# junejunejune/c_orb_slam

Measured on AMD Instinct MI355X. Metric: tracking FPS + ORB matches/sec, KITTI-00 stereo; local-BA iter/sec, higher is better.
Workload: dtype u8

## Files before the change

### c_orb_slam_amd/csrc/ba.hpp

```cpp
#pragma once
#include <functional>
#include <hip/hip_runtime.h>

#include <cstdint>
#include <future>
#include <vector>

#include "../../include/orbslam_gpu.h"
#include "ba_struct.hpp"
#include "ba_struct_gpu.hpp"
#include "ba_types.hpp"
#include "comm.hpp"
#include "ldlt.hpp"
#include "orb_common.hpp"

namespace orbgpu {

constexpr int kBaTiledMinPoses = 24;

struct Se3 {
    double q[4];
    double t[3];
    double pad;
};
// ... 146 lines not shown
struct PoseProbDev;
class PoseEngine {
public:
    ~PoseEngine();
    int init();
    int run(int count, const pose_problem* P, float* Tcw_out, uint8_t* const* outlier, int* ninliers);
    int run_device(int count, const pose_problem* P, float* const* Tcw_out, uint8_t* const* outlier, int* ninliers);
    int run_frames_device(int count, const pose_frame* F, float* const* Tcw_out, uint8_t* const* outlier,
                          int* ninliers, hipStream_t s = nullptr, DeferredChain* chain = nullptr);
    hipStream_t stream() const { return stream_; }
    void set_timing(bool on) { timing_ = on; }
    int last_timing(float* ms);

private:
    int launch_device(int count, const int* Ns, const std::function<void(int, PoseProbDev&)>& fill,
                      float* const* Tcw_out, uint8_t* const* outlier, int* ninliers, hipStream_t s = nullptr,
                      DeferredChain* chain = nullptr);
    hipStream_t stream_ = nullptr;
    void* dArena_ = nullptr;
    void* hArena_ = nullptr;
    size_t cap_ = 0;
    hipEvent_t lastUse_ = nullptr;
    bool lastUseSet_ = false;
    bool timing_ = false, timed_ = false;
    hipEvent_t tA_ = nullptr, tB_ = nullptr;
};

int debug_ldlt(int n, const double* S, const double* b, double* x, int variant);
int debug_csum(const double* v, int n, double* out);
int debug_ldlt_factor(int n, const double* S, double* out);
int debug_wave_tree(const double* v64, double* out);
int debug_shared_div(const double* a, const double* b, int n, double* out);
int debug_set_csum_lds_max(int v);
int debug_set_scale_small_max(int v);
int debug_set_struct_gpu_min_edges(int v);
int debug_set_posegraph_check(int on);
int debug_prof(unsigned long long* out32);

}
```

### c_orb_slam_amd/csrc/capi_match.cpp

```cpp
#include <cstring>
#include <new>
#include <vector>

#include "capi_handles.hpp"

using orbgpu::FrameDev;
using orbgpu::Matcher;
using orbgpu::SearchDev;


namespace {

size_t al(size_t n) { return (n + 255) & ~(size_t)255; }

template <class T>
T* up(Matcher* m, const T* src, size_t count, hipStream_t s, int* err) {
    if (!src || count == 0) return nullptr;
    void* d = m->arena_alloc(count * sizeof(T));
    if (!d || hipMemcpyAsync(d, src, count * sizeof(T), hipMemcpyHostToDevice, s) != hipSuccess) {
        *err = ORB_E_HIP;
        return nullptr;
    }
    return (T*)d;
}
// ... 319 lines not shown
        f.projX = proj_x[p];
        f.projXR = proj_xr[p];
        f.projY = proj_y[p];
        f.level = level[p];
        f.viewCos = view_cos[p];
        f.mpIndex = (int*)m->arena_alloc((size_t)std::max(maps[p].n, 1) * 4);
        f.nvisible = d_nv + p;
        if (!f.mpIndex) return ORB_E_HIP;
    }
    if (err) return err;
    if (m->frustum(probs, fr, viewingCosLimit, logScaleFactor)) return ORB_E_HIP;
    if (hipMemcpyAsync(nvisible, d_nv, (size_t)count * 4, hipMemcpyDeviceToHost, s) != hipSuccess) return ORB_E_HIP;
    return orbgpu::stream_wait(s) == hipSuccess ? ORB_OK : ORB_E_HIP;
}

int ORBmatcher_SearchLocalPoints_batch(ORBmatcher_h h, int count, const orb_frame* F, int32_t* const* cur_mp,
                                       const orb_localmap* maps, float logScaleFactor, float th, float nnratio,
                                       int* nmatches, int* nvisible) {
    if (!h || count < 0 || (count > 0 && (!F || !cur_mp || !maps || !nmatches || !nvisible))) return ORB_E_INVALID;
    if (count == 0) return ORB_OK;
    Matcher* m = h->m;
    if (!m->device_pointers()) return ORB_E_INVALID;
    hipStream_t s = m->stream();
    size_t need = al((size_t)count * 8) + al(sizeof(orbgpu::FrustumDev) * count) + 4096;
    for (int p = 0; p < count; p++) {
        const orb_localmap& M = maps[p];
        if (!frame_ok(&F[p]) || !F[p].Tcw || M.n < 0 || !cur_mp[p]) return ORB_E_INVALID;
        if (M.n > 0 && (!M.pos || !M.desc || !M.observations || !M.max_dist || !M.min_dist || !M.normal || !M.skip))
            return ORB_E_INVALID;
        need += 7 * al((size_t)M.n * 4) + 256;
    }
    if (m->arena_reserve(need)) return ORB_E_HIP;
    int err = 0;
    int* d_cnt = (int*)m->count_buf((size_t)count * 8);
    if (!d_cnt) return ORB_E_HIP;
    if (hipMemsetAsync(d_cnt, 0, (size_t)count * 8, s) != hipSuccess) return ORB_E_HIP;
    std::vector<SearchDev> probs(count);
    std::vector<orbgpu::FrustumDev> fr(count);
    for (int p = 0; p < count; p++) {
        SearchDev& P = probs[p];
        memset(&P, 0, sizeof(P));
        P.cur = frame_dev(m, &F[p], true, s, &err);
        P.nq = maps[p].n;
        P.mpPos = maps[p].pos;
        P.mpDesc = maps[p].desc;
        P.mpObs = maps[p].observations;
        P.curMP = cur_mp[p];
        P.nmatches = d_cnt + p;
        orbgpu::FrustumDev& f = fr[p];
        memset(&f, 0, sizeof(f));
        f.maxDist = maps[p].max_dist;
        f.minDist = maps[p].min_dist;
        f.normal = maps[p].normal;
        f.skip = maps[p].skip;
        f.nvisible = d_cnt + count + p;
    }
    if (err) return err;
    const int rc = m->search_local_points(probs, fr, 0.5f, logScaleFactor, th, nnratio > 0.f ? nnratio : m->nnratio());
    if (rc) return rc == -1 ? ORB_E_INVALID : ORB_E_HIP;
    if (m->d2h_counts(nmatches, d_cnt, (size_t)count * 4) || m->d2h_counts(nvisible, d_cnt + count, (size_t)count * 4))
        return ORB_E_HIP;
    (void)s;
    return m->end_call() ? ORB_E_HIP : ORB_OK;
}

int ORBmatcher_SearchDense_batch(ORBmatcher_h h, int count, const uint8_t* const* qdesc, const int* nq,
                                 const uint8_t* const* tdesc, const int* nt, int32_t* const* best_idx,
                                 int32_t* const* best_dist, int32_t* const* second_dist) {
    if (!h || count < 0 || (count > 0 && (!qdesc || !nq || !tdesc || !nt || !best_idx || !best_dist || !second_dist)))
        return ORB_E_INVALID;
    for (int p = 0; p < count; p++) {
        if (nq[p] < 0 || nt[p] < 0) return ORB_E_INVALID;
        if (nq[p] > 0 && (!qdesc[p] || !best_idx[p] || !best_dist[p] || !second_dist[p])) return ORB_E_INVALID;
        if (nt[p] > 0 && !tdesc[p]) return ORB_E_INVALID;
    }
    if (count == 0) return ORB_OK;
    Matcher* m = h->m;
    const bool dev = m->device_pointers();
    hipStream_t s = m->stream();
    std::vector<orbgpu::DenseDev> probs;
    if (!dev) {
        size_t need = 4096;
// ... 89 lines not shown
```

### c_orb_slam_amd/csrc/capi_stereo.cpp

```cpp
#include <algorithm>
#include <cmath>
#include <cstring>
#include <vector>

#include "capi_handles.hpp"
#include "stereo.hpp"

namespace {
size_t al(size_t n) { return (n + 255) & ~(size_t)255; }

template <class T>
T* up(orbgpu::Matcher* m, const T* src, size_t count, hipStream_t s, int* err) {
    if (!src || count == 0) return nullptr;
    void* d = m->arena_alloc(count * sizeof(T));
    if (!d || hipMemcpyAsync(d, src, count * sizeof(T), hipMemcpyHostToDevice, s) != hipSuccess) {
        *err = ORB_E_HIP;
        return nullptr;
    }
    return (T*)d;
}
}

extern "C" {

// ... 15 lines not shown
        !keysR || !descR || !uRight || !depth || !nmatches)
        return ORB_E_INVALID;
    if (npairs == 0) return ORB_OK;
    const orbgpu::Extractor* EL = left->ex;
    const orbgpu::Extractor* ER = right->ex;
    if (!EL->pyramid_base() || !ER->pyramid_base() || first_left + npairs > EL->last_batch() ||
        first_right + npairs > ER->last_batch())
        return ORB_E_INVALID;
    const auto& LL = EL->levels();
    const auto& LR = ER->levels();
    if (LL.size() != LR.size() || (int)LL.size() > orbgpu::kStereoMaxLevels) return ORB_E_INVALID;
    for (size_t l = 0; l < LL.size(); l++)
        if (LL[l].w != LR[l].w || LL[l].h != LR[l].h || LL[l].pitch != LR[l].pitch || LL[l].off != LR[l].off)
            return ORB_E_INVALID;
    if (!(mb > 0.0f)) return ORB_E_INVALID;
    for (int p = 0; p < npairs; p++) {
        if (NL[p] < 0 || NR[p] < 0 || NL[p] > orbgpu::kStereoMaxKeys || NR[p] > 65535) return ORB_E_INVALID;
        if ((NL[p] && (!keysL[p] || !descL[p] || !uRight[p] || !depth[p])) || (NR[p] && (!keysR[p] || !descR[p])))
            return ORB_E_INVALID;
    }
    orbgpu::Matcher* m = h->m;
    const bool dev = m->device_pointers();
    hipStream_t s = m->stream();
    if (orbgpu::stream_wait(EL->stream()) != hipSuccess ||
        (ER != EL && orbgpu::stream_wait(ER->stream()) != hipSuccess))
        return ORB_E_HIP;
    orbgpu::StereoParams P;
    std::memset(&P, 0, sizeof(P));
    for (size_t l = 0; l < LL.size(); l++) {
        P.lv[l].off = (long long)LL[l].off;
        P.lv[l].pitch = LL[l].pitch;
        P.lv[l].w = LL[l].w;
        P.lv[l].h = LL[l].h;
        P.scale[l] = EL->scale()[l];
        P.invScale[l] = EL->inv_scale()[l];
    }
    P.mbf = mbf;
    P.mb = mb;
    P.rows0 = LL[0].h;
    if (P.rows0 > orbgpu::kStereoMaxRows) return ORB_E_INVALID;
    const int band = (int)std::ceil(4.0f * EL->scale()[LL.size() - 1]) + 3;
    size_t need = al(sizeof(orbgpu::StereoDev) * npairs) + al(4 * (size_t)npairs);
    int maxNL = 0;
    for (int p = 0; p < npairs; p++) {
        need += al(4 * (size_t)NL[p]) + al(4 * ((size_t)P.rows0 + 1)) + al(8 * (size_t)NR[p] * band + 8);
        if (!dev) need += al(28 * (size_t)NL[p]) + al(32 * (size_t)NL[p]) + al(28 * (size_t)NR[p]) +
                          al(32 * (size_t)NR[p]) + 2 * al(4 * (size_t)NL[p]);
        maxNL = std::max(maxNL, NL[p]);
// ... 240 lines not shown
```

### c_orb_slam_amd/csrc/orb_common.hpp

```cpp
#pragma once
#include <hip/hip_runtime.h>
#include <cstdint>
#include <cstdio>
#include <cstring>
#include <deque>
#include <mutex>
#include <vector>

#define ORB_HIP_CHECK(expr)                                                            \
    do {                                                                               \
        hipError_t _e = (expr);                                                        \
        if (_e != hipSuccess) {                                                        \
            fprintf(stderr, "[orbslam_gpu] HIP error %s at %s:%d: %s\n",               \
                    hipGetErrorName(_e), __FILE__, __LINE__, #expr);                   \
            return -2;                                                                 \
        }                                                                              \
    } while (0)

namespace orbgpu {

hipError_t stream_wait(hipStream_t s);

class DeferredChain {
public:
    ~DeferredChain() {
        for (auto& b : blocks_) (void)hipHostFree(b.p);
        for (auto& b : devs_) (void)hipFree(b.p);
        for (auto& e : events_)
            if (e.ev) (void)hipEventDestroy(e.ev);
    }
    bool on() const { return on_; }
    void set(bool v) { on_ = v; }
    void* stage(const void* src, size_t bytes) {
        void* p = take(bytes);
        if (p && bytes) std::memcpy(p, src, bytes);
        return p;
    }
    void* land(void* user, size_t bytes) {
        void* p = take(bytes);
        if (p) cur_outs_.push_back(Out{p, user, bytes});
        return p;
    }
    void* dev_counts(size_t bytes) {
        bytes = (bytes + 255) & ~(size_t)255;
        std::lock_guard<std::mutex> g(mu_);
        if (cur_dev_ < 0 || devs_[cur_dev_].used + bytes > devs_[cur_dev_].cap) {
            int k = -1;
            for (size_t q = 0; q < devs_.size(); q++)
                if (!devs_[q].busy && devs_[q].cap >= bytes) {
                    k = (int)q;
                    break;
                }
            if (k < 0) {
                void* p = nullptr;
                const size_t cap = bytes < 65536 ? 65536 : bytes;
                if (hipMalloc(&p, cap) != hipSuccess) return nullptr;
                devs_.push_back(DevBlock{p, cap, 0, false});
                k = (int)devs_.size() - 1;
            }
            devs_[k].busy = true;
            devs_[k].used = 0;
            cur_devs_.push_back(k);
            cur_dev_ = k;
        }
        DevBlock& b = devs_[cur_dev_];
        void* p = (char*)b.p + b.used;
        b.used += bytes;
        return p;
    }
    void land_dev(void* user, const void* dev, size_t bytes) {
        std::lock_guard<std::mutex> g(mu_);
        cur_dev_outs_.push_back(DevOut{user, dev, bytes});
    }
    int close(hipStream_t s, long long* id) {
        std::vector<int> devs;
        std::vector<DevOut> douts;
        std::vector<DevBlock> snap;
        {
            std::lock_guard<std::mutex> g(mu_);
            devs.swap(cur_devs_);
            douts.swap(cur_dev_outs_);
            cur_dev_ = -1;
            for (int k : devs) snap.push_back(devs_[k]);
        }
        bool ok = true;
        std::vector<Out> mapped;
        for (const DevBlock& b : snap) {
            if (!b.used) continue;
            char* pin = (char*)take(b.used);
            if (!pin || hipMemcpyAsync(pin, b.p, b.used, hipMemcpyDeviceToHost, s) != hipSuccess) {
                ok = false;
                break;
            }
            for (const DevOut& o : douts)
                if ((const char*)o.dev >= (const char*)b.p && (const char*)o.dev < (const char*)b.p + b.cap)
                    mapped.push_back(Out{pin + ((const char*)o.dev - (const char*)b.p), o.user, o.bytes});
        }
        std::lock_guard<std::mutex> g(mu_);
        size_t k = 0;
        if (ok) {
            while (k < events_.size() && (events_[k].live || events_[k].waiters > 0)) k++;
            if (k == events_.size()) {
                events_.push_back(Ev{});
                ok = hipEventCreateWithFlags(&events_[k].ev, hipEventDisableTiming) == hipSuccess;
            }
            ok = ok && hipEventRecord(events_[k].ev, s) == hipSuccess;
        }
        if (!ok) {
            fprintf(stderr, "[orbslam_gpu] deferred chain: closing the epoch failed; its counts are lost\n");
            (void)hipStreamSynchronize(s);
            for (int d : devs) devs_[d].busy = false;
            for (int b : cur_blocks_) blocks_[b].busy = false;
            cur_blocks_.clear();
            cur_outs_.clear();
            failed_ = true;
            return -2;
        }
        for (auto& o : mapped) cur_outs_.push_back(o);
        events_[k].live = true;
// ... 61 lines not shown

private:
    struct Block {
        void* p;
        size_t cap;
        bool busy;
    };
    struct Out {
        void* pin;
        void* user;
        size_t bytes;
    };
    struct Epoch {
        long long id;
        int ev;
        std::vector<int> blocks;
        std::vector<Out> outs;
        std::vector<int> devs;
    };
    struct DevBlock {
        void* p;
        size_t cap, used;
        bool busy;
    };
    struct DevOut {
        void* user;
        const void* dev;
        size_t bytes;
    };
    struct Ev {
        hipEvent_t ev = nullptr;
        bool live = false;
        int waiters = 0;
    };
    void* take(size_t bytes) {
        bytes = (bytes + 255) & ~(size_t)255;
        std::lock_guard<std::mutex> g(mu_);
        for (size_t k = 0; k < blocks_.size(); k++)
            if (!blocks_[k].busy && blocks_[k].cap >= bytes) {
                blocks_[k].busy = true;
                cur_blocks_.push_back((int)k);
                return blocks_[k].p;
            }
        void* p = nullptr;
        const size_t cap = bytes < 65536 ? 65536 : bytes;
        if (hipHostMalloc(&p, cap) != hipSuccess) return nullptr;
// ... 162 lines not shown
```

### c_orb_slam_amd/csrc/orb_extract.hip

```cpp
#include "orb_extract.hpp"

#include <algorithm>
#include <atomic>
#include <chrono>
#include <cmath>
#include <cstring>
#include <thread>

namespace orbgpu {

__constant__ int8_t c_pattern[256 * 4];
__constant__ int8_t c_disc[2 * 1024];
__constant__ int c_ndisc;
__constant__ int c_umax[16];
__constant__ int c_gauss[7];

static const int8_t kPattern[256 * 4] = {
#include "brief_pattern.inc"
};

__device__ __forceinline__ int xcd_tile(int bid, int nb) { return (bid & 7) * (nb >> 3) + (bid >> 3); }
static inline unsigned grid8(int n) { return (unsigned)((n + 7) & ~7); }
constexpr int kFastSplitLevel = 3;

// ... 1497 lines not shown
    selcap_ = jcap_ * nlevels_;
    ORB_HIP_CHECK(hipMalloc(&d_octlv_, ol.size() * sizeof(OctLevelDev)));
    ORB_HIP_CHECK(hipMemcpy(d_octlv_, ol.data(), ol.size() * sizeof(OctLevelDev), hipMemcpyHostToDevice));
    ORB_HIP_CHECK(hipMalloc(&d_jobsel_, (size_t)B * nlevels_ * jcap_ * 4));
    ORB_HIP_CHECK(hipMalloc(&d_jobcnt_, (size_t)B * nlevels_ * 4));
    ORB_HIP_CHECK(hipMalloc(&d_gscr_, (size_t)packed_cap_ * 3 * 2));
    ORB_HIP_CHECK(hipMalloc(&d_nout_, (size_t)(B + 1) * 4));
    ORB_HIP_CHECK(hipFree(d_sel_));
    d_sel_ = nullptr;
    sel_cap_ = selcap_ * B;
    ORB_HIP_CHECK(hipMalloc(&d_sel_, (size_t)sel_cap_ * sizeof(int2)));
    if (h_nout_) (void)hipHostFree(h_nout_);
    ORB_HIP_CHECK(hipHostMalloc((void**)&h_nout_, (size_t)(B + 1) * 4));
    geomW_ = W;
    geomH_ = H;
    return 0;
}

int Extractor::extract(const uint8_t* imgs, int B, int W, int H, int step, size_t img_stride,
                       bool imgs_on_device, orb_kp* kps, uint8_t* desc, int cap, bool out_on_device,
                       int* n_out, const uint8_t* const* list) {
    if (B <= 0 || B > maxB_ || W <= 0 || H <= 0) return -1;
    if (W > maxW_ || H > maxH_) return -1;
    if (int e = setup_geometry(W, H)) return e;
    hipStream_t s = stream_;
    const uint8_t* src = imgs;
    if (!imgs_on_device) {
        const size_t need = img_stride * (B - 1) + (size_t)step * (H - 1) + W;
        if (need > in_cap_) {
            if (d_in_) (void)hipFree(d_in_);
            ORB_HIP_CHECK(hipMalloc(&d_in_, need));
            in_cap_ = need;
        }
        if (h_in_) ORB_HIP_CHECK(hipEventSynchronize(ev_[0]));
        if (need > h_in_cap_) {
            if (h_in_) (void)hipHostFree(h_in_);
            h_in_ = nullptr;
            h_in_cap_ = 0;
            ORB_HIP_CHECK(hipHostMalloc(&h_in_, need));
            h_in_cap_ = need;
        }
        if (list) {
            const size_t one = (size_t)step * (H - 1) + W;
            for (int b = 0; b < B; b++) std::memcpy((uint8_t*)h_in_ + img_stride * b, list[b], one);
        } else {
            std::memcpy(h_in_, imgs, need);
// ... 127 lines not shown
                           (const int*)d_nout_, levelArgs_, okps, odesc, cap, gx, B);
    }
    ORB_HIP_CHECK(hipGetLastError());
    ORB_HIP_CHECK(hipMemcpyAsync(h_nout_, d_nout_, (size_t)(B + 1) * 4, hipMemcpyDeviceToHost, s));
    ORB_HIP_CHECK(hipEventRecord(ev_[6], s));
    ORB_HIP_CHECK(stream_wait(s));
    const int err = h_nout_[B];
    for (int b = 0; b < B; b++) n_out[b] = h_nout_[b];
    if (err & 1) return -3;
    if (err) return -1;
    if (!out_on_device) {
        for (int b = 0; b < B; b++) {
            if (n_out[b] == 0) continue;
            ORB_HIP_CHECK(hipMemcpyAsync(kps + (size_t)b * cap, okps + (size_t)b * cap, (size_t)n_out[b] * sizeof(orb_kp_dev),
                                         hipMemcpyDeviceToHost, s));
            ORB_HIP_CHECK(hipMemcpyAsync(desc + (size_t)b * cap * 32, odesc + (size_t)b * cap * 32, (size_t)n_out[b] * 32,
                                         hipMemcpyDeviceToHost, s));
        }
        ORB_HIP_CHECK(stream_wait(s));
    }
    last_B_ = B;
    planFlags_ = planFlags;
    planChainFrom_ = planChainFrom;
    return 0;
}

int Extractor::last_plan(int* flags, int* chain_from, int* tile_rows) const {
    if (last_B_ <= 0) return -1;
    if (flags) *flags = planFlags_;
    if (chain_from) *chain_from = planChainFrom_;
    if (tile_rows)
        for (int i = 0; i < 2 * nlevels_; i++) tile_rows[i] = ptile_th_[i];
    return 0;
}

int Extractor::corner_total(long long* total) {
    if (last_B_ <= 0 || !d_gtotal_) return -1;
    int v = 0;
    ORB_HIP_CHECK(hipStreamSynchronize(stream_));
    ORB_HIP_CHECK(hipMemcpy(&v, d_gtotal_, 4, hipMemcpyDeviceToHost));
    *total = v;
    return 0;
}

int Extractor::get_blurred(int index, int level, uint8_t* dst, int dst_step, int* w, int* h) {
    if (level < 0 || level >= nlevels_ || index < 0 || index >= last_B_ || !d_blur_) return -1;
// ... 46 lines not shown
```

### c_orb_slam_amd/csrc/orb_extract.hpp

```cpp
#pragma once
#include <atomic>
#include <condition_variable>
#include <cstddef>
#include <cstdint>
#include <mutex>
#include <thread>
#include <vector>
#include <array>

#include "orb_common.hpp"
#include "octree.hpp"
#include "../../include/orbslam_gpu.h"

namespace orbgpu {

struct orb_kp_dev {
    float x, y, size, angle, response;
    int32_t octave, class_id;
};
static_assert(sizeof(orb_kp_dev) == 28, "cv::KeyPoint layout");

struct CellDesc {
    int r0, r1, c0, c1;
    int offx, offy;
// ... 51 lines not shown

constexpr int kPlanFlow = 1, kPlanChain = 2, kPlanFastSplit = 4, kPlanBlurSide = 8, kPlanBlurEarly = 16,
              kPlanTile32 = 32;

struct LevelHost {
    int w, h, pw, ph, pitch, bpitch;
    size_t off, boff;
};

class Extractor {
public:
    Extractor(int nfeatures, float scaleFactor, int nlevels, int iniTh, int minTh);
    ~Extractor();
    int init_device(int maxW, int maxH, int maxBatch);
    int extract(const uint8_t* imgs, int B, int W, int H, int step, size_t img_stride, bool imgs_on_device,
                orb_kp* kps, uint8_t* desc, int cap, bool out_on_device, int* n_out,
                const uint8_t* const* list = nullptr);
    int get_level(int index, int level, uint8_t* dst, int dst_step, int* w, int* h);
    int get_blurred(int index, int level, uint8_t* dst, int dst_step, int* w, int* h);
    int timings(float* ms6);
    int corner_total(long long* total);
    int last_plan(int* flags, int* chain_from, int* tile_rows) const;
    hipStream_t stream() const { return stream_; }
    int reserve_cus(int one_in_n);
    int share_stream(Extractor* with);
    int build_work(int B);
    const uint8_t* pyramid_base() const { return (const uint8_t*)d_pyr_; }
    size_t pyramid_image_bytes() const { return img_bytes_; }
    const std::vector<LevelHost>& levels() const { return levels_; }
    int last_batch() const { return last_B_; }

    int nlevels() const { return nlevels_; }
    float scale_factor() const { return scaleFactor_; }
    const std::vector<float>& scale() const { return scale_; }
    const std::vector<float>& inv_scale() const { return invScale_; }
    const std::vector<float>& sigma2() const { return sigma2_; }
    const std::vector<float>& inv_sigma2() const { return invSigma2_; }
    const std::vector<int>& n_per_level() const { return nPerLevel_; }

private:
    static void gaussian_taps(int taps[7]);
    int setup_geometry(int W, int H);
    void release();

    int nfeatures_;
    double scaleFactorD_;
// ... 14 lines not shown
    std::vector<int> ptile_begin_, ptile_n_, plds_;
    std::vector<int> ptile_th_;
    bool flow_ = false;
    int* d_flowcnt_ = nullptr;
    int flowBands_[2] = {0, 0}, flowLds_[2] = {0, 0};
    FlowArgs flow_args(int v, int B) const;
    int plan_chain(const std::vector<std::vector<int>>& yr);
    bool chain_ = false;
    int chainK_ = 0, chainLds_ = 0, chainFrom_ = 0, chainSrcLds_ = 0, chainSrcRp_ = 0;
    std::vector<std::vector<int>> xofsAll_;
    std::vector<std::vector<short>> xalAll_;
    size_t chainStripOff_ = 0, chainRowOff_ = 0;
    std::vector<uint8_t> chainTab_;
    void* d_chain_ = nullptr;
    void* d_cellslot_ = nullptr;
    std::vector<std::array<size_t, 4>> tab_off_;
    size_t img_bytes_ = 0, blur_bytes_ = 0, slots_per_image_ = 0;
    int packed_cap_ = 0, sel_cap_ = 0;
    int last_B_ = 0;
    int planFlags_ = 0, planChainFrom_ = 0;

    hipStream_t stream_ = nullptr;
    bool ownStream_ = true;
    int lent_ = 0;
    hipEvent_t ev_[7] = {};
    hipStream_t side_ = nullptr;
    hipEvent_t evBlur_ = nullptr;
    bool fastSplit_ = false;
    hipEvent_t evPyrA_ = nullptr, evFastA_ = nullptr;
    void *d_in_ = nullptr, *d_pyr_ = nullptr, *d_blur_ = nullptr, *d_slots_ = nullptr, *d_counts_ = nullptr;
    void *d_ptiles_ = nullptr;
    void *d_cells_ = nullptr, *d_tiles_ = nullptr, *d_lcb_ = nullptr, *d_packed_ = nullptr, *d_hdr_ = nullptr;
    void *d_sel_ = nullptr, *d_levels_ = nullptr, *d_tabs_ = nullptr, *d_kps_ = nullptr, *d_desc_ = nullptr;
    int* d_gtotal_ = nullptr;
    void* d_work_ = nullptr;
    void* d_groups_ = nullptr;
    int work_B_ = -1, work_n_ = 0;
    int work_part_[2] = {0, 0};
    bool d_gtotal_alias_ = false;
    size_t in_cap_ = 0, out_cap_ = 0;
    void* h_in_ = nullptr;
    size_t h_in_cap_ = 0;
    void *d_jobsel_ = nullptr, *d_jobcnt_ = nullptr, *d_octlv_ = nullptr, *d_gscr_ = nullptr, *d_nout_ = nullptr;
    int jcap_ = 0, selcap_ = 0;
    int* h_nout_ = nullptr;

// ... 6 lines not shown
```

### c_orb_slam_amd/csrc/orb_match.hip

```cpp
#define ORBGPU_PROF_BLOCK 20
#include "orb_match.hpp"

#include <chrono>
#include <cstdlib>

#include <cstring>

#include "detmath.hpp"

namespace orbgpu {

constexpr int TH_HIGH = 100;
constexpr int kSelectLocalThreads = 1024;
constexpr int HISTO_LENGTH = 30;

__device__ __forceinline__ int hamming32(const uint8_t* a, const uint8_t* b) {
    const uint4* pa = reinterpret_cast<const uint4*>(a);
    const uint4* pb = reinterpret_cast<const uint4*>(b);
    const uint4 a0 = pa[0], a1 = pa[1], b0 = pb[0], b1 = pb[1];
    return __popc(a0.x ^ b0.x) + __popc(a0.y ^ b0.y) + __popc(a0.z ^ b0.z) + __popc(a0.w ^ b0.w) +
           __popc(a1.x ^ b1.x) + __popc(a1.y ^ b1.y) + __popc(a1.z ^ b1.z) + __popc(a1.w ^ b1.w);
}

struct Desc32 {
// ... 998 lines not shown
    if (arena_used_ + bytes > arena_cap_) return nullptr;
    void* p = (char*)d_arena_ + arena_used_;
    arena_used_ += bytes;
    return p;
}

static inline int cand_gx(int maxq, int nt) { return (maxq + nt - 1) / nt; }
static inline dim3 cand_grid(int maxq, int nt, int np) { return xcd_grid(cand_gx(maxq, nt), np); }

int Matcher::run(std::vector<SearchDev>& probs, float th, bool bMono, bool lastMode, float nnratio) {
    const int np = (int)probs.size();
    if (np == 0) return 0;
    size_t need = 0;
    int maxq = 0, maxN = 1;
    const bool vis = frustum_ != nullptr;
    for (auto& p : probs) {
        if (p.cur.N > kMaxFrameKeys || p.cur.N < 0 || p.nq < 0) return -1;
        maxN = std::max(maxN, p.cur.N);
        need += ((size_t)(kGridCells + 1 + p.cur.N) * 4 + 255) & ~(size_t)255;
        need += ((size_t)p.nq * (kTopK * 8 + 16 + 8) + 255) & ~(size_t)255;
        if (vis) need += ((size_t)p.nq * 4 + 255) & ~(size_t)255;
        maxq = std::max(maxq, p.nq);
    }
    if (vis) need += ((size_t)np * 4 + 255) & ~(size_t)255;
    if (need > scratch_cap_) {
        if (d_scratch_) (void)hipFree(d_scratch_);
        scratch_cap_ = need * 2;
        ORB_HIP_CHECK(hipMalloc(&d_scratch_, scratch_cap_));
    }
    char* s = (char*)d_scratch_;
    int* visCounts = nullptr;
    if (vis) {
        visCounts = (int*)s;
        s += ((size_t)np * 4 + 255) & ~(size_t)255;
    }
    for (size_t k = 0; k < probs.size(); k++) {
        SearchDev& p = probs[k];
        p.gridStart = (int*)s;
        p.gridIdx = p.gridStart + kGridCells + 1;
        s += ((size_t)(kGridCells + 1 + p.cur.N) * 4 + 255) & ~(size_t)255;
        p.topk = (int2*)s;
        p.qinfo = (int4*)(p.topk + (size_t)p.nq * kTopK);
        p.hist = (int2*)(p.qinfo + p.nq);
        s += ((size_t)p.nq * (kTopK * 8 + 16 + 8) + 255) & ~(size_t)255;
        p.visList = nullptr;
        p.visCount = nullptr;
        if (vis) {
            p.visList = (int*)s;
            p.visCount = visCounts + k;
            s += ((size_t)p.nq * 4 + 255) & ~(size_t)255;
        }
    }
    if (vis) ORB_HIP_CHECK(hipMemsetAsync(visCounts, 0, (size_t)np * 4, stream_));
    const size_t pb = sizeof(SearchDev) * np;
    if (pb > probs_cap_) {
        if (d_probs_) (void)hipFree(d_probs_);
        probs_cap_ = pb * 2;
        ORB_HIP_CHECK(hipMalloc(&d_probs_, probs_cap_));
    }
    ORB_HIP_CHECK(hipMemcpyAsync(d_probs_, h2d_src(probs.data(), pb), pb, hipMemcpyHostToDevice, stream_));
    SearchDev* dp = (SearchDev*)d_probs_;
    if (frustum_ && maxq > 0) {
        mark(8);
        hipLaunchKernelGGL(k_frustum, cand_grid(maxq, 256, np), dim3(256), 0, stream_, (const SearchDev*)dp,
                           frustum_, frustumCos_, frustumLsf_, np, cand_gx(maxq, 256));
        mark(9);
    }
    if (timing_) {
        if (int e = zero_counters(0, 2)) return e;
        mark(0);
    }
    hipLaunchKernelGGL(k_build_grid, dim3(np), dim3(256), grid_lds_bytes(maxN), stream_, dp, 1);
    mark(1);
    if (maxq > 0) {
        if (lastMode) {
            if (maxN <= kStageMaxN && stage_threads() == 256)
                hipLaunchKernelGGL((k_candidates<true, true, 256>), cand_grid(maxq, 256, np), dim3(256), kStageLds,
                                   stream_, dp, np, cand_gx(maxq, 256), th, (int)bMono, counters());
            else if (maxN <= kStageMaxN)
                hipLaunchKernelGGL((k_candidates<true, true, kStageThreads>), cand_grid(maxq, kStageThreads, np),
                                   dim3(kStageThreads), kStageLds,
                                   stream_, dp, np, cand_gx(maxq, kStageThreads), th, (int)bMono, counters());
            else
                hipLaunchKernelGGL((k_candidates<true, false, 256>), cand_grid(maxq, 256, np), dim3(256), 0, stream_, dp,
// ... 37 lines not shown
    const int np = (int)probs.size();
    int maxq = 0;
    for (auto& p : probs) maxq = std::max(maxq, p.nq);
    if (np == 0 || maxq == 0) return 0;
    const size_t pb = sizeof(SearchDev) * np;
    if (pb > probs_cap_) {
        if (d_probs_) (void)hipFree(d_probs_);
        probs_cap_ = pb * 2;
        ORB_HIP_CHECK(hipMalloc(&d_probs_, probs_cap_));
    }
    FrustumDev* dfr = (FrustumDev*)arena_alloc(sizeof(FrustumDev) * np);
    if (!dfr) return -2;
    ORB_HIP_CHECK(hipMemcpyAsync(d_probs_, probs.data(), pb, hipMemcpyHostToDevice, stream_));
    ORB_HIP_CHECK(hipMemcpyAsync(dfr, fr.data(), sizeof(FrustumDev) * np, hipMemcpyHostToDevice, stream_));
    mark(8);
    hipLaunchKernelGGL(k_frustum, cand_grid(maxq, 256, np), dim3(256), 0, stream_, (const SearchDev*)d_probs_, dfr,
                       viewingCosLimit, logScaleFactor, np, cand_gx(maxq, 256));
    mark(9);
    ORB_HIP_CHECK(hipGetLastError());
    return 0;
}

int Matcher::search_local_points(std::vector<SearchDev>& probs, std::vector<FrustumDev>& fr, float viewingCosLimit,
                                 float logScaleFactor, float th, float nnratio) {
    const int np = (int)probs.size();
    if (np == 0) return 0;
    int maxq = 0;
    for (auto& p : probs) maxq = std::max(maxq, p.nq);
    if (maxq > 0) {
        size_t need = sizeof(FrustumDev) * np + 256;
        for (auto& p : probs) need += 7 * ((((size_t)p.nq * 4) + 255) & ~(size_t)255);
        char* base = (char*)arena_alloc(need);
        if (!base) return -2;
        char* o = base + ((sizeof(FrustumDev) * np + 255) & ~(size_t)255);
        for (int k = 0; k < np; k++) {
            const size_t b = (((size_t)probs[k].nq * 4) + 255) & ~(size_t)255;
            FrustumDev& f = fr[k];
            f.inView = (uint8_t*)o; o += b;
            f.projX = (float*)o; o += b;
            f.projXR = (float*)o; o += b;
            f.projY = (float*)o; o += b;
            f.level = (int*)o; o += b;
            f.viewCos = (float*)o; o += b;
            f.mpIndex = (int*)o; o += b;
            SearchDev& P = probs[k];
            P.inView = f.inView; P.projX = f.projX; P.projXR = f.projXR; P.projY = f.projY;
            P.level = f.level; P.viewCos = f.viewCos; P.mpIndex = f.mpIndex;
        }
        ORB_HIP_CHECK(hipMemcpyAsync(base, h2d_src(fr.data(), sizeof(FrustumDev) * np), sizeof(FrustumDev) * np,
                                     hipMemcpyHostToDevice, stream_));
        frustum_ = (const FrustumDev*)base;
        frustumCos_ = viewingCosLimit;
        frustumLsf_ = logScaleFactor;
    }
    const int rc = run(probs, th, false, false, nnratio);
    frustum_ = nullptr;
    return rc;
}
int Matcher::search_local(std::vector<SearchDev>& probs, float th) { return run(probs, th, false, false, nnratio_); }

int Matcher::candidates(const uint8_t* q, int nq, const uint8_t* t, int nt, const int* off, const int* cand, int* dist,
                        int* best_idx, int* best_dist, int* second_dist) {
    (void)nt;
    if (nq <= 0) return 0;
    if (timing_) {
        if (int e = zero_counters(4, 2)) return e;
        mark(12);
    }
    hipLaunchKernelGGL(k_csr_hamming, dim3((nq + 3) / 4), dim3(256), 0, stream_, q, nq, t, off, cand, dist, best_idx,
                       best_dist, second_dist, counters());
    mark(13);
    ORB_HIP_CHECK(hipGetLastError());
    return 0;
}

static int dense_block() {
    static const int v = [] {
        const char* e = std::getenv("ORBGPU_DENSE_TB");
        const int b = e ? std::atoi(e) : kDenseBlock;
// ... 137 lines not shown
```

### c_orb_slam_amd/csrc/orb_match.hpp

```cpp
#pragma once
#include <cstdint>
#include <vector>

#include "orb_common.hpp"
#include "orb_extract.hpp"

namespace orbgpu {

constexpr int kGridCols = 64;
constexpr int kGridRows = 48;
constexpr int kGridCells = kGridCols * kGridRows;
constexpr int kTopK = 8;
constexpr int kMaxFrameKeys = 4096;

struct FrameDev {
    int N;
    const orb_kp_dev* keysUn;
    const uint8_t* desc;
    const float* uRight;
    float minX, maxX, minY, maxY, gridWInv, gridHInv;
    const float* scale;
    int nlevels;
    float fx, fy, cx, cy, bf, b;
    const float* Tcw;
// ... 49 lines not shown
    int* best_idx;
    int* best_dist;
    int* second_dist;
};

struct AreaQuery {
    float x, y, r;
    int minLevel, maxLevel;
    int qd;
};

constexpr int kCountSlots = 64;

class Matcher {
public:
    Matcher(float nnratio, bool checkOri) : nnratio_(nnratio), checkOri_(checkOri) {}
    ~Matcher();
    int init_device();
    void set_device_pointers(bool on) { device_ptrs_ = on; }
    bool device_pointers() const { return device_ptrs_; }
    int search_last(std::vector<SearchDev>& probs, float th, bool bMono);
    int search_local(std::vector<SearchDev>& probs, float th);
    int search_local_points(std::vector<SearchDev>& probs, std::vector<FrustumDev>& fr, float viewingCosLimit,
                            float logScaleFactor, float th, float nnratio);
    int frustum(std::vector<SearchDev>& probs, const std::vector<FrustumDev>& fr, float viewingCosLimit,
                float logScaleFactor);
    int candidates(const uint8_t* q, int nq, const uint8_t* t, int nt, const int* off, const int* cand, int* dist,
                   int* best_idx, int* best_dist, int* second_dist);
    int dense(const std::vector<DenseDev>& probs);
    int dense_timing(float* ms, long long* pairs);
    hipStream_t stream() const { return stream_; }
    DeferredChain& chain() { return chain_; }
    const void* h2d_src(const void* host, size_t bytes) { return chain_.on() ? chain_.stage(host, bytes) : host; }
    void* count_buf(size_t bytes) { return chain_.on() ? chain_.dev_counts(bytes) : arena_alloc(bytes); }
    int d2h_counts(void* user, const void* dev, size_t bytes) {
        if (chain_.on()) {
            chain_.land_dev(user, dev, bytes);
            return 0;
        }
        ORB_HIP_CHECK(hipMemcpyAsync(user, dev, bytes, hipMemcpyDeviceToHost, stream_));
        return 0;
    }
    int end_call() {
        if (chain_.on()) return 0;
        ORB_HIP_CHECK(hipStreamSynchronize(stream_));
        return 0;
    }
    float nnratio() const { return nnratio_; }
    bool check_ori() const { return checkOri_; }

    int area_candidates(const SearchDev& frame, const AreaQuery* d_q, int nq, const uint8_t* d_qdesc,
                        std::vector<int>& off, std::vector<int2>& cand);
    int arena_reserve(size_t bytes);
    void* arena_alloc(size_t bytes);

    int set_timing(bool on);
    bool timing() const { return timing_; }
// ... 2 lines not shown
    unsigned long long* counters() const { return timing_ ? d_count_ : nullptr; }
    int zero_counters(int first, int n);

private:
    int run(std::vector<SearchDev>& probs, float th, bool bMono, bool lastMode, float nnratio);
    float nnratio_;
    bool checkOri_;
    bool device_ptrs_ = false;
    hipStream_t stream_ = nullptr;
    DeferredChain chain_;
    void* d_scratch_ = nullptr;
    size_t scratch_cap_ = 0;
    void* d_probs_ = nullptr;
    size_t probs_cap_ = 0;
    void* d_arena_ = nullptr;
    size_t arena_cap_ = 0, arena_used_ = 0;
    void* d_cand_ = nullptr;
    size_t cand_cap_ = 0;
    void* d_dense_ = nullptr;
    size_t dense_cap_ = 0;
    bool timing_ = false;
    const FrustumDev* frustum_ = nullptr;
    float frustumCos_ = 0.5f, frustumLsf_ = 0.f;
    hipEvent_t ev_[16] = {};
    bool evSet_[16] = {};
    unsigned long long* d_count_ = nullptr;
};

int debug_prof_match(unsigned long long* out32);

}
```

### c_orb_slam_amd/csrc/pose_opt.hip

```cpp
#include <algorithm>
#include <cstdlib>
#include <cstring>
#include <functional>
#include <vector>

#include "ba.hpp"
#include "ba_math.hpp"
#include "orb_common.hpp"

namespace orbgpu {

struct PoseEdgeDev {
    float Xw[3], obs[3];
    float info;
    int meta;
};

struct PoseProbDev {
    int ne, e0;
    int nbad, N;
    Se3 T0;
    Se3 T;
    double fx, fy, cx, cy, bf;
    const float* Tcw;
// ... 859 lines not shown
    if (!dNin) return -2;
    std::vector<PoseProbDev> tmp;
    PoseProbDev* hp = (PoseProbDev*)hArena_;
    if (chain) {
        tmp.resize(count);
        hp = tmp.data();
    }
    size_t e0 = 0;
    for (int f = 0; f < count; f++) {
        PoseProbDev& pp = hp[f];
        memset(&pp, 0, sizeof(pp));
        pp.N = Ns[f];
        pp.e0 = (int)e0;
        e0 += (size_t)std::min(Ns[f], kPoseMaxEdges + 1);
        fill(f, pp);
        pp.Tcw_out = Tcw_out[f];
        pp.outlier = outlier[f];
        pp.ninl = dNin + f;
    }
    PoseProbDev* dp = (PoseProbDev*)d;
    PoseEdgeDev* dE = (PoseEdgeDev*)(d + bProb);
    const void* src = chain ? chain->stage(hp, sizeof(PoseProbDev) * count) : (const void*)hp;
    if (!src) return -2;
    if (lastUseSet_) ORB_HIP_CHECK(hipStreamWaitEvent(st, lastUse_, 0));
    ORB_HIP_CHECK(hipMemcpyAsync(d, src, sizeof(PoseProbDev) * count, hipMemcpyHostToDevice, st));
    hipLaunchKernelGGL(k_pose_pack, dim3(count), dim3(kPackThreads), 0, st, dp, dE);
    if (timing_) ORB_HIP_CHECK(hipEventRecord(tA_, st));
    if (count <= pose_wide_max())
        hipLaunchKernelGGL(k_pose_opt<kPoseThreadsWide>, dim3(count), dim3(kPoseThreadsWide),
                           pose_lds_pad((const void*)k_pose_opt<kPoseThreadsWide>), st, dp, (const PoseEdgeDev*)dE,
                           nullptr, (uint8_t*)(d + bProb + bEdge));
    else
        hipLaunchKernelGGL(k_pose_opt<kPoseThreads>, dim3(count), dim3(kPoseThreads),
                           pose_lds_pad((const void*)k_pose_opt<kPoseThreads>), st, dp, (const PoseEdgeDev*)dE, nullptr,
                           (uint8_t*)(d + bProb + bEdge));
    ORB_HIP_CHECK(hipGetLastError());
    if (timing_) {
        ORB_HIP_CHECK(hipEventRecord(tB_, st));
        timed_ = true;
    }
    if (chain) {
        chain->land_dev(ninliers, dNin, sizeof(int) * count);
        ORB_HIP_CHECK(hipEventRecord(lastUse_, st));
        lastUseSet_ = true;
        return 0;
    }
    ORB_HIP_CHECK(hipMemcpyAsync(hp, d, bProb, hipMemcpyDeviceToHost, st));
    ORB_HIP_CHECK(hipEventRecord(lastUse_, st));
    lastUseSet_ = true;
    ORB_HIP_CHECK(stream_wait(st));
    int rc = 0;
    for (int f = 0; f < count; f++) {
        const PoseProbDev& pp = hp[f];
        if (pp.ne < 0) rc = -3;
        ninliers[f] = pp.ne < 0 || pp.nbad < 0 ? 0 : pp.ne - pp.nbad;
    }
    return rc;
}

int PoseEngine::last_timing(float* ms) {
    if (!timed_) return -1;
    ORB_HIP_CHECK(hipEventSynchronize(tB_));
    ORB_HIP_CHECK(hipEventElapsedTime(ms, tA_, tB_));
    return 0;
}

PoseEngine::~PoseEngine() {
    if (lastUseSet_) (void)hipEventSynchronize(lastUse_);
    if (lastUse_) (void)hipEventDestroy(lastUse_);
    if (tA_) (void)hipEventDestroy(tA_);
    if (tB_) (void)hipEventDestroy(tB_);
    if (dArena_) (void)hipFree(dArena_);
// ... 56 lines not shown
                e.Xw[j] = Q.Xw[3 * i + j];
                e.obs[j] = Q.obs[3 * i + j];
            }
            e.info = Q.inv_sigma2[i];
            e.meta = i | (!(Q.obs[3 * i + 2] < 0) ? (int)0x80000000u : 0);
        }
    }
    PoseProbDev* dp = (PoseProbDev*)d;
    ORB_HIP_CHECK(hipMemcpyAsync(d, h, bProb + sizeof(PoseEdgeDev) * ne, hipMemcpyHostToDevice, stream_));
    if (count > 0)
    {
        if (count <= pose_wide_max())
            hipLaunchKernelGGL(k_pose_opt<kPoseThreadsWide>, dim3(count), dim3(kPoseThreadsWide), 0, stream_, dp, (const PoseEdgeDev*)(d + bProb),
                               (double*)(d + bProb + bEdge), (uint8_t*)(d + bProb + bEdge + bErr));
        else
            hipLaunchKernelGGL(k_pose_opt<kPoseThreads>, dim3(count), dim3(kPoseThreads), 0, stream_, dp, (const PoseEdgeDev*)(d + bProb),
                               (double*)(d + bProb + bEdge), (uint8_t*)(d + bProb + bEdge + bErr));
    }
    ORB_HIP_CHECK(hipGetLastError());
    ORB_HIP_CHECK(hipMemcpyAsync(h, d, bProb, hipMemcpyDeviceToHost, stream_));
    if (ne) ORB_HIP_CHECK(hipMemcpyAsync(hOut, d + bProb + bEdge + bErr, ne, hipMemcpyDeviceToHost, stream_));
    ORB_HIP_CHECK(hipEventRecord(lastUse_, stream_));
    lastUseSet_ = true;
    ORB_HIP_CHECK(hipStreamSynchronize(stream_));
    for (int f = 0; f < count; f++) {
        const pose_problem& Q = P[f];
        const PoseProbDev& pp = hp[f];
        const uint8_t* o = hOut + pp.e0;
        for (int i = 0, k = 0; i < Q.N; i++)
            if (Q.has_mp[i]) {
                outlier[f][i] = pp.nbad < 0 ? 0 : o[k];
                k++;
            }
        if (pp.nbad < 0) {
            memcpy(Tcw_out + 16 * (size_t)f, Q.Tcw, sizeof(float) * 16);
            ninliers[f] = 0;
        } else {
            host_se3_to_Tcw(pp.T, Tcw_out + 16 * (size_t)f);
            ninliers[f] = pp.ne - pp.nbad;
        }
    }
    return 0;
}

}
```

Before: 44570.

## Pack local-point search buffers into one upload region and skip redundant syncs

Counts, visibility counters, frustum descriptors and search problems for local-point search now share one contiguous device region. They are zero-filled on the host and uploaded with a single H2D copy, which replaces the separate memsets and copies. Deferred-chain count readback now copies only the registered ranges instead of whole blocks. The change also skips stream waits when the extractor is idle and skips the pose event wait when the last use was on the same stream. These changes cut API calls and sync overhead, at the cost of more bookkeeping and a risk of race bugs from the idle flag.

Result: no change. 44390 (-0.4%).

```diff
diff --git a/c_orb_slam_amd/csrc/ba.hpp b/c_orb_slam_amd/csrc/ba.hpp
--- a/c_orb_slam_amd/csrc/ba.hpp
+++ b/c_orb_slam_amd/csrc/ba.hpp
@@ -192,6 +192,7 @@
     size_t cap_ = 0;
     hipEvent_t lastUse_ = nullptr;
     bool lastUseSet_ = false;
+    hipStream_t lastUseStream_ = nullptr;
     bool timing_ = false, timed_ = false;
     hipEvent_t tA_ = nullptr, tB_ = nullptr;
 };
diff --git a/c_orb_slam_amd/csrc/capi_match.cpp b/c_orb_slam_amd/csrc/capi_match.cpp
--- a/c_orb_slam_amd/csrc/capi_match.cpp
+++ b/c_orb_slam_amd/csrc/capi_match.cpp
@@ -365,7 +365,8 @@
     Matcher* m = h->m;
     if (!m->device_pointers()) return ORB_E_INVALID;
     hipStream_t s = m->stream();
-    size_t need = al((size_t)count * 8) + al(sizeof(orbgpu::FrustumDev) * count) + 4096;
+    size_t need = al((size_t)count * 8) + al((size_t)count * 4) + al(sizeof(orbgpu::FrustumDev) * count) +
+                  al(sizeof(SearchDev) * count) + 4096;
     for (int p = 0; p < count; p++) {
         const orb_localmap& M = maps[p];
         if (!frame_ok(&F[p]) || !F[p].Tcw || M.n < 0 || !cur_mp[p]) return ORB_E_INVALID;
@@ -375,9 +376,7 @@
     }
     if (m->arena_reserve(need)) return ORB_E_HIP;
     int err = 0;
-    int* d_cnt = (int*)m->count_buf((size_t)count * 8);
-    if (!d_cnt) return ORB_E_HIP;
-    if (hipMemsetAsync(d_cnt, 0, (size_t)count * 8, s) != hipSuccess) return ORB_E_HIP;
+    int* d_cnt = nullptr;
     std::vector<SearchDev> probs(count);
     std::vector<orbgpu::FrustumDev> fr(count);
     for (int p = 0; p < count; p++) {
@@ -389,18 +388,18 @@
         P.mpDesc = maps[p].desc;
         P.mpObs = maps[p].observations;
         P.curMP = cur_mp[p];
-        P.nmatches = d_cnt + p;
         orbgpu::FrustumDev& f = fr[p];
         memset(&f, 0, sizeof(f));
         f.maxDist = maps[p].max_dist;
         f.minDist = maps[p].min_dist;
         f.normal = maps[p].normal;
         f.skip = maps[p].skip;
-        f.nvisible = d_cnt + count + p;
     }
     if (err) return err;
-    const int rc = m->search_local_points(probs, fr, 0.5f, logScaleFactor, th, nnratio > 0.f ? nnratio : m->nnratio());
+    const int rc = m->search_local_points(probs, fr, 0.5f, logScaleFactor, th, nnratio > 0.f ? nnratio : m->nnratio(),
+                                          &d_cnt);
     if (rc) return rc == -1 ? ORB_E_INVALID : ORB_E_HIP;
+    if (!d_cnt) return ORB_E_HIP;
     if (m->d2h_counts(nmatches, d_cnt, (size_t)count * 4) || m->d2h_counts(nvisible, d_cnt + count, (size_t)count * 4))
         return ORB_E_HIP;
     (void)s;
diff --git a/c_orb_slam_amd/csrc/capi_stereo.cpp b/c_orb_slam_amd/csrc/capi_stereo.cpp
--- a/c_orb_slam_amd/csrc/capi_stereo.cpp
+++ b/c_orb_slam_amd/csrc/capi_stereo.cpp
@@ -61,8 +61,8 @@
     orbgpu::Matcher* m = h->m;
     const bool dev = m->device_pointers();
     hipStream_t s = m->stream();
-    if (orbgpu::stream_wait(EL->stream()) != hipSuccess ||
-        (ER != EL && orbgpu::stream_wait(ER->stream()) != hipSuccess))
+    if ((!EL->idle() && orbgpu::stream_wait(EL->stream()) != hipSuccess) ||
+        (ER != EL && !ER->idle() && orbgpu::stream_wait(ER->stream()) != hipSuccess))
         return ORB_E_HIP;
     orbgpu::StereoParams P;
     std::memset(&P, 0, sizeof(P));
diff --git a/c_orb_slam_amd/csrc/orb_common.hpp b/c_orb_slam_amd/csrc/orb_common.hpp
--- a/c_orb_slam_amd/csrc/orb_common.hpp
+++ b/c_orb_slam_amd/csrc/orb_common.hpp
@@ -41,8 +41,9 @@
         if (p) cur_outs_.push_back(Out{p, user, bytes});
         return p;
     }
-    void* dev_counts(size_t bytes) {
+    void* dev_counts(size_t bytes, size_t copy_bytes = ~(size_t)0) {
         bytes = (bytes + 255) & ~(size_t)255;
+        copy_bytes = copy_bytes >= bytes ? bytes : (copy_bytes + 255) & ~(size_t)255;
         std::lock_guard<std::mutex> g(mu_);
         if (cur_dev_ < 0 || devs_[cur_dev_].used + bytes > devs_[cur_dev_].cap) {
             int k = -1;
@@ -55,16 +56,23 @@
                 void* p = nullptr;
                 const size_t cap = bytes < 65536 ? 65536 : bytes;
                 if (hipMalloc(&p, cap) != hipSuccess) return nullptr;
-                devs_.push_back(DevBlock{p, cap, 0, false});
+                devs_.push_back(DevBlock{p, cap, 0, false, {}});
                 k = (int)devs_.size() - 1;
             }
             devs_[k].busy = true;
             devs_[k].used = 0;
+            devs_[k].ranges.clear();
             cur_devs_.push_back(k);
             cur_dev_ = k;
         }
         DevBlock& b = devs_[cur_dev_];
         void* p = (char*)b.p + b.used;
+        if (copy_bytes) {
+            if (!b.ranges.empty() && b.ranges.back().first + b.ranges.back().second == b.used)
+                b.ranges.back().second += copy_bytes;
+            else
+                b.ranges.push_back({b.used, copy_bytes});
+        }
         b.used += bytes;
         return p;
     }
@@ -86,15 +94,18 @@
         bool ok = true;
         std::vector<Out> mapped;
         for (const DevBlock& b : snap) {
-            if (!b.used) continue;
-            char* pin = (char*)take(b.used);
-            if (!pin || hipMemcpyAsync(pin, b.p, b.used, hipMemcpyDeviceToHost, s) != hipSuccess) {
-                ok = false;
-                break;
-            }
-            for (const DevOut& o : douts)
-                if ((const char*)o.dev >= (const char*)b.p && (const char*)o.dev < (const char*)b.p + b.cap)
-                    mapped.push_back(Out{pin + ((const char*)o.dev - (const char*)b.p), o.user, o.bytes});
+            for (const auto& r : b.ranges) {
+                const char* d0 = (const char*)b.p + r.first;
+                char* pin = (char*)take(r.second);
+                if (!pin || hipMemcpyAsync(pin, d0, r.second, hipMemcpyDeviceToHost, s) != hipSuccess) {
+                    ok = false;
+                    break;
+                }
+                for (const DevOut& o : douts)
+                    if ((const char*)o.dev >= d0 && (const char*)o.dev < d0 + r.second)
+                        mapped.push_back(Out{pin + ((const char*)o.dev - d0), o.user, o.bytes});
+            }
+            if (!ok) break;
         }
         std::lock_guard<std::mutex> g(mu_);
         size_t k = 0;
@@ -202,6 +213,7 @@
         void* p;
         size_t cap, used;
         bool busy;
+        std::vector<std::pair<size_t, size_t>> ranges;
     };
     struct DevOut {
         void* user;
diff --git a/c_orb_slam_amd/csrc/orb_extract.hip b/c_orb_slam_amd/csrc/orb_extract.hip
--- a/c_orb_slam_amd/csrc/orb_extract.hip
+++ b/c_orb_slam_amd/csrc/orb_extract.hip
@@ -1543,6 +1543,7 @@
                        int* n_out, const uint8_t* const* list) {
     if (B <= 0 || B > maxB_ || W <= 0 || H <= 0) return -1;
     if (W > maxW_ || H > maxH_) return -1;
+    idle_.store(false, std::memory_order_release);
     if (int e = setup_geometry(W, H)) return e;
     hipStream_t s = stream_;
     const uint8_t* src = imgs;
@@ -1716,6 +1717,7 @@
     last_B_ = B;
     planFlags_ = planFlags;
     planChainFrom_ = planChainFrom;
+    idle_.store(true, std::memory_order_release);
     return 0;
 }
 
diff --git a/c_orb_slam_amd/csrc/orb_extract.hpp b/c_orb_slam_amd/csrc/orb_extract.hpp
--- a/c_orb_slam_amd/csrc/orb_extract.hpp
+++ b/c_orb_slam_amd/csrc/orb_extract.hpp
@@ -97,6 +97,7 @@
     int corner_total(long long* total);
     int last_plan(int* flags, int* chain_from, int* tile_rows) const;
     hipStream_t stream() const { return stream_; }
+    bool idle() const { return idle_.load(std::memory_order_acquire); }
     int reserve_cus(int one_in_n);
     int share_stream(Extractor* with);
     int build_work(int B);
@@ -157,6 +158,7 @@
 
     hipStream_t stream_ = nullptr;
     bool ownStream_ = true;
+    std::atomic<bool> idle_{true};
     int lent_ = 0;
     hipEvent_t ev_[7] = {};
     hipStream_t side_ = nullptr;
diff --git a/c_orb_slam_amd/csrc/orb_match.hip b/c_orb_slam_amd/csrc/orb_match.hip
--- a/c_orb_slam_amd/csrc/orb_match.hip
+++ b/c_orb_slam_amd/csrc/orb_match.hip
@@ -1044,18 +1044,13 @@
         if (vis) need += ((size_t)p.nq * 4 + 255) & ~(size_t)255;
         maxq = std::max(maxq, p.nq);
     }
-    if (vis) need += ((size_t)np * 4 + 255) & ~(size_t)255;
     if (need > scratch_cap_) {
         if (d_scratch_) (void)hipFree(d_scratch_);
         scratch_cap_ = need * 2;
         ORB_HIP_CHECK(hipMalloc(&d_scratch_, scratch_cap_));
     }
     char* s = (char*)d_scratch_;
-    int* visCounts = nullptr;
-    if (vis) {
-        visCounts = (int*)s;
-        s += ((size_t)np * 4 + 255) & ~(size_t)255;
-    }
+    int* visCounts = vis ? (int*)(region_.dev + region_.cnt) : nullptr;
     for (size_t k = 0; k < probs.size(); k++) {
         SearchDev& p = probs[k];
         p.gridStart = (int*)s;
@@ -1073,15 +1068,26 @@
             s += ((size_t)p.nq * 4 + 255) & ~(size_t)255;
         }
     }
-    if (vis) ORB_HIP_CHECK(hipMemsetAsync(visCounts, 0, (size_t)np * 4, stream_));
     const size_t pb = sizeof(SearchDev) * np;
-    if (pb > probs_cap_) {
-        if (d_probs_) (void)hipFree(d_probs_);
-        probs_cap_ = pb * 2;
-        ORB_HIP_CHECK(hipMalloc(&d_probs_, probs_cap_));
-    }
-    ORB_HIP_CHECK(hipMemcpyAsync(d_probs_, h2d_src(probs.data(), pb), pb, hipMemcpyHostToDevice, stream_));
-    SearchDev* dp = (SearchDev*)d_probs_;
+    SearchDev* dp = nullptr;
+    if (region_.dev) {
+        const size_t o = region_.cnt + region_.vis;
+        h_region_.assign(region_.total, 0);
+        std::memcpy(h_region_.data() + o, regionFr_->data(), sizeof(FrustumDev) * np);
+        std::memcpy(h_region_.data() + o + region_.fr, probs.data(), pb);
+        const void* src = h2d_src(h_region_.data(), region_.total);
+        if (!src) return -2;
+        ORB_HIP_CHECK(hipMemcpyAsync(region_.dev, src, region_.total, hipMemcpyHostToDevice, stream_));
+        dp = (SearchDev*)(region_.dev + o + region_.fr);
+    } else {
+        if (pb > probs_cap_) {
+            if (d_probs_) (void)hipFree(d_probs_);
+            probs_cap_ = pb * 2;
+            ORB_HIP_CHECK(hipMalloc(&d_probs_, probs_cap_));
+        }
+        ORB_HIP_CHECK(hipMemcpyAsync(d_probs_, h2d_src(probs.data(), pb), pb, hipMemcpyHostToDevice, stream_));
+        dp = (SearchDev*)d_probs_;
+    }
     if (frustum_ && maxq > 0) {
         mark(8);
         hipLaunchKernelGGL(k_frustum, cand_grid(maxq, 256, np), dim3(256), 0, stream_, (const SearchDev*)dp,
@@ -1165,17 +1171,30 @@
 }
 
 int Matcher::search_local_points(std::vector<SearchDev>& probs, std::vector<FrustumDev>& fr, float viewingCosLimit,
-                                 float logScaleFactor, float th, float nnratio) {
+                                 float logScaleFactor, float th, float nnratio, int** d_counts) {
     const int np = (int)probs.size();
     if (np == 0) return 0;
     int maxq = 0;
     for (auto& p : probs) maxq = std::max(maxq, p.nq);
+    const auto al = [](size_t b) { return (b + 255) & ~(size_t)255; };
+    LocalRegion R;
+    R.cnt = al((size_t)np * 8);
+    R.vis = al((size_t)np * 4);
+    R.fr = al(sizeof(FrustumDev) * np);
+    R.total = R.cnt + R.vis + R.fr + sizeof(SearchDev) * np;
+    R.dev = (char*)count_buf(R.total, R.cnt);
+    if (!R.dev) return -2;
+    int* d_cnt = (int*)R.dev;
+    for (int k = 0; k < np; k++) {
+        probs[k].nmatches = d_cnt + k;
+        fr[k].nvisible = d_cnt + np + k;
+    }
+    *d_counts = d_cnt;
     if (maxq > 0) {
-        size_t need = sizeof(FrustumDev) * np + 256;
+        size_t need = 256;
         for (auto& p : probs) need += 7 * ((((size_t)p.nq * 4) + 255) & ~(size_t)255);
-        char* base = (char*)arena_alloc(need);
-        if (!base) return -2;
-        char* o = base + ((sizeof(FrustumDev) * np + 255) & ~(size_t)255);
+        char* o = (char*)arena_alloc(need);
+        if (!o) return -2;
         for (int k = 0; k < np; k++) {
             const size_t b = (((size_t)probs[k].nq * 4) + 255) & ~(size_t)255;
             FrustumDev& f = fr[k];
@@ -1190,14 +1209,16 @@
             P.inView = f.inView; P.projX = f.projX; P.projXR = f.projXR; P.projY = f.projY;
             P.level = f.level; P.viewCos = f.viewCos; P.mpIndex = f.mpIndex;
         }
-        ORB_HIP_CHECK(hipMemcpyAsync(base, h2d_src(fr.data(), sizeof(FrustumDev) * np), sizeof(FrustumDev) * np,
-                                     hipMemcpyHostToDevice, stream_));
-        frustum_ = (const FrustumDev*)base;
+        frustum_ = (const FrustumDev*)(R.dev + R.cnt + R.vis);
         frustumCos_ = viewingCosLimit;
         frustumLsf_ = logScaleFactor;
     }
+    region_ = R;
+    regionFr_ = &fr;
     const int rc = run(probs, th, false, false, nnratio);
     frustum_ = nullptr;
+    region_ = LocalRegion{};
+    regionFr_ = nullptr;
     return rc;
 }
 int Matcher::search_local(std::vector<SearchDev>& probs, float th) { return run(probs, th, false, false, nnratio_); }
diff --git a/c_orb_slam_amd/csrc/orb_match.hpp b/c_orb_slam_amd/csrc/orb_match.hpp
--- a/c_orb_slam_amd/csrc/orb_match.hpp
+++ b/c_orb_slam_amd/csrc/orb_match.hpp
@@ -95,7 +95,7 @@
     int search_last(std::vector<SearchDev>& probs, float th, bool bMono);
     int search_local(std::vector<SearchDev>& probs, float th);
     int search_local_points(std::vector<SearchDev>& probs, std::vector<FrustumDev>& fr, float viewingCosLimit,
-                            float logScaleFactor, float th, float nnratio);
+                            float logScaleFactor, float th, float nnratio, int** d_counts);
     int frustum(std::vector<SearchDev>& probs, const std::vector<FrustumDev>& fr, float viewingCosLimit,
                 float logScaleFactor);
     int candidates(const uint8_t* q, int nq, const uint8_t* t, int nt, const int* off, const int* cand, int* dist,
@@ -105,7 +105,9 @@
     hipStream_t stream() const { return stream_; }
     DeferredChain& chain() { return chain_; }
     const void* h2d_src(const void* host, size_t bytes) { return chain_.on() ? chain_.stage(host, bytes) : host; }
-    void* count_buf(size_t bytes) { return chain_.on() ? chain_.dev_counts(bytes) : arena_alloc(bytes); }
+    void* count_buf(size_t bytes, size_t copy_bytes = ~(size_t)0) {
+        return chain_.on() ? chain_.dev_counts(bytes, copy_bytes) : arena_alloc(bytes);
+    }
     int d2h_counts(void* user, const void* dev, size_t bytes) {
         if (chain_.on()) {
             chain_.land_dev(user, dev, bytes);
@@ -154,6 +156,13 @@
     bool timing_ = false;
     const FrustumDev* frustum_ = nullptr;
     float frustumCos_ = 0.5f, frustumLsf_ = 0.f;
+    struct LocalRegion {
+        char* dev = nullptr;
+        size_t cnt = 0, vis = 0, fr = 0, total = 0;
+    };
+    LocalRegion region_;
+    const std::vector<FrustumDev>* regionFr_ = nullptr;
+    std::vector<char> h_region_;
     hipEvent_t ev_[16] = {};
     bool evSet_[16] = {};
     unsigned long long* d_count_ = nullptr;
diff --git a/c_orb_slam_amd/csrc/pose_opt.hip b/c_orb_slam_amd/csrc/pose_opt.hip
--- a/c_orb_slam_amd/csrc/pose_opt.hip
+++ b/c_orb_slam_amd/csrc/pose_opt.hip
@@ -905,7 +905,7 @@
     PoseEdgeDev* dE = (PoseEdgeDev*)(d + bProb);
     const void* src = chain ? chain->stage(hp, sizeof(PoseProbDev) * count) : (const void*)hp;
     if (!src) return -2;
-    if (lastUseSet_) ORB_HIP_CHECK(hipStreamWaitEvent(st, lastUse_, 0));
+    if (lastUseSet_ && lastUseStream_ != st) ORB_HIP_CHECK(hipStreamWaitEvent(st, lastUse_, 0));
     ORB_HIP_CHECK(hipMemcpyAsync(d, src, sizeof(PoseProbDev) * count, hipMemcpyHostToDevice, st));
     hipLaunchKernelGGL(k_pose_pack, dim3(count), dim3(kPackThreads), 0, st, dp, dE);
     if (timing_) ORB_HIP_CHECK(hipEventRecord(tA_, st));
@@ -926,11 +926,13 @@
         chain->land_dev(ninliers, dNin, sizeof(int) * count);
         ORB_HIP_CHECK(hipEventRecord(lastUse_, st));
         lastUseSet_ = true;
+        lastUseStream_ = st;
         return 0;
     }
     ORB_HIP_CHECK(hipMemcpyAsync(hp, d, bProb, hipMemcpyDeviceToHost, st));
     ORB_HIP_CHECK(hipEventRecord(lastUse_, st));
     lastUseSet_ = true;
+    lastUseStream_ = st;
     ORB_HIP_CHECK(stream_wait(st));
     int rc = 0;
     for (int f = 0; f < count; f++) {
@@ -1033,6 +1035,7 @@
     if (ne) ORB_HIP_CHECK(hipMemcpyAsync(hOut, d + bProb + bEdge + bErr, ne, hipMemcpyDeviceToHost, stream_));
     ORB_HIP_CHECK(hipEventRecord(lastUse_, stream_));
     lastUseSet_ = true;
+    lastUseStream_ = stream_;
     ORB_HIP_CHECK(hipStreamSynchronize(stream_));
     for (int f = 0; f < count; f++) {
         const pose_problem& Q = P[f];
```
